# yoseph007/PQA2

Measured on AMD Instinct MI355X. Metric: VMAF frames/sec (vif+adm+motion2 -> SVM), device-resident synthetic YUV pairs, higher is better.
Workload: dtype f32; 1 GPU; 2160p 3840x2160 8-bit, vmaf_4k_v0.6.1, 300 frames/GPU; frames_per_gpu=300, frames_total=300, batch=97, frames_per_launch=75, clips_pipelined=True, parallelism=frame-shard x1, 1-frame motion halo, all-gather of records + of scores

## Files before the change

pqa2_amd/csrc/kernels.h:

```cpp
#pragma once
#include <hip/hip_runtime.h>
#include <stdint.h>

#include <vector>

namespace pqa {

enum Elem : int { ELEM_U8 = 0, ELEM_U16 = 1, ELEM_F32 = 2 };

struct PlaneRun {
  const void* base;
  int64_t row_pitch;
  int64_t frame_pitch;
};

struct MutPlaneRun {
  void* base;
  int64_t row_pitch;
  int64_t frame_pitch;
};

int vif_tile_w(int scale);
constexpr int kVifTileH = 8;
inline int vif_tiles_x(int scale, int w) { return (w + vif_tile_w(scale) - 1) / vif_tile_w(scale); }
inline int vif_tiles_y(int h) { return (h + kVifTileH - 1) / kVifTileH; }

enum : int { VIF_S0_VALU = 0, VIF_S0_AUTO = 1 };
hipError_t launch_vif_stat(hipStream_t stream, int scale, Elem elem, PlaneRun ref, PlaneRun dis, int n_frames,
                           int w, int h, float inv_scale, float gain_limit, int border101, double* partials,
                           MutPlaneRun next_ref, MutPlaneRun next_dis, int s0_mode = VIF_S0_AUTO, int* n_partials = nullptr,
                           int uniform = 1);
hipError_t vif_march_prepare();
int vif_march_partials_max(int w, int h);
int vif_march_table(uint16_t* out, int capacity_halfwords);
void vif_march_shape(int w, int h, int* out6);
bool launch_vif_s0_march(hipStream_t stream, Elem elem, int bits, PlaneRun ref, PlaneRun dis, int n_frames, int w, int h, float gain_limit,
                         int border101, double* partials, MutPlaneRun next_ref, MutPlaneRun next_dis, int* n_partials,
                         hipError_t* err, int uniform = 1);
constexpr int kVifFxPartials = 8;
void vif_fixed_log2_table(uint16_t* out32768);
hipError_t launch_vif_fixed(hipStream_t stream, int scale, int bit_depth, Elem elem, PlaneRun ref, PlaneRun dis,
                            int n_frames, int w, int h, double gain_limit, const uint16_t* log2_lut,
                            long long* partials, MutPlaneRun next_ref, MutPlaneRun next_dis);

constexpr int kAdmTileW = 60, kAdmTileH = 14;
inline int adm_tiles_x(int band_w) { return (band_w + kAdmTileW - 1) / kAdmTileW; }
inline int adm_tiles_y(int band_h) { return (band_h + kAdmTileH - 1) / kAdmTileH; }

enum : int { ADM_TILED = 0, ADM_AUTO = 1, ADM_MARCH = 2 };
hipError_t launch_adm_scale(hipStream_t stream, int scale, Elem elem, PlaneRun ref, PlaneRun dis, int n_frames,
                            int w, int h, float inv_scale, float gain_limit, MutPlaneRun ll_ref,
                            MutPlaneRun ll_dis, double* partials, int mode = ADM_AUTO, int* n_partials = nullptr);
int adm_march_partials(int band_w, int band_h);
bool launch_adm_march(hipStream_t stream, int scale, Elem elem, PlaneRun ref, PlaneRun dis, int n_frames, int w, int h,
                      float inv_scale, float gain_limit, MutPlaneRun ll_ref, MutPlaneRun ll_dis, double* partials,
                      int* n_partials, hipError_t* err);
bool adm_pyramid_takes(Elem elem, int w, int h);
int adm_pyramid_partials(int w, int h);
bool launch_adm_pyramid(hipStream_t stream, Elem elem, PlaneRun ref, PlaneRun dis, int n_frames, int w, int h, float inv_scale,
                        float gain_limit, MutPlaneRun ll_ref, MutPlaneRun ll_dis, double* partials0, double* partials1,
                        int* n_partials, hipError_t* err);
float adm_dwt_quant_step(int lambda, int theta);

constexpr int kAdmFxRows = kAdmTileH + 2;
struct AdmFxScale {
  int scale, band_w, band_h;
  int left, top, right, bottom;
  float rf[3];
  uint32_t i_rf[3];
  int cm_shift_sq[3], cm_shift_sub[3], cm_shift_cub[3], cm_final_q[3];
  int den_shift_sq, den_shift_cub, den_final_q;
  int num_row_shift, den_row_shift;
};
AdmFxScale adm_fixed_scale_params(int scale, int band_w, int band_h);
void adm_fixed_div_table(int32_t* out65537);
void adm_fixed_epilogue(const AdmFxScale& p, const long long acc[6], double* num_out, double* den_out);
hipError_t launch_adm_fixed(hipStream_t stream, int scale, int bit_depth, Elem elem, PlaneRun ref, PlaneRun dis,
                            int n_frames, int w, int h, double gain_limit, const int32_t* div_lut,
                            MutPlaneRun ll_ref, MutPlaneRun ll_dis, long long* partials);

constexpr int kMotionTileW = 252, kMotionTileH = 16;
inline int motion_tiles(int w, int h) {
  return ((w + kMotionTileW - 1) / kMotionTileW) * ((h + kMotionTileH - 1) / kMotionTileH);
}
enum : int { MOTION_TILED = 0, MOTION_AUTO = 1 };
hipError_t launch_motion(hipStream_t stream, Elem elem, PlaneRun ref, const void* prev0, int64_t prev0_row_pitch,
                         int n_frames, int w, int h, float inv_scale, double* partials, int mode = MOTION_AUTO,
                         int* n_partials = nullptr);
int motion_march_partials(int w, int h);
bool launch_motion_march(hipStream_t stream, Elem elem, PlaneRun ref, const void* prev0, int64_t prev0_row_pitch, int n_frames,
                         int w, int h, double* partials, int* n_partials, hipError_t* err);
hipError_t launch_motion_fixed(hipStream_t stream, int bit_depth, Elem elem, PlaneRun ref, const void* prev0,
                               int64_t prev0_row_pitch, int n_frames, int w, int h, unsigned long long* partials);

constexpr int kSseBlocksPerPlane = 256;
hipError_t launch_sse(hipStream_t stream, Elem elem, PlaneRun a, PlaneRun b, int n_frames, int w, int h,
                      unsigned long long* partials);

constexpr int kSsimTileBW = 32, kSsimTileBH = 8;
inline int ssim_tiles(int w, int h) {
  const int ww = (w >> 2) - 1, wh = (h >> 2) - 1;
  if (ww < 1 || wh < 1) return 0;
  return ((ww + kSsimTileBW - 1) / kSsimTileBW) * ((wh + kSsimTileBH - 1) / kSsimTileBH);
}
hipError_t launch_ssim(hipStream_t stream, Elem elem, PlaneRun main, PlaneRun ref, int n_frames, int w, int h,
                       int max_value, double* partials, unsigned long long* sse_partials);

constexpr int kLumaBlocks = 128;
hipError_t launch_luma_stats(hipStream_t stream, Elem elem, PlaneRun luma, int n_frames, int w, int h,
                             unsigned threshold, int gray_bit_depth, unsigned long long* partials,
                             unsigned long long* out);
void luma_gray_map(int bit_depth, float* a, float* b);

struct FinalizeArgs {
// ... 261 lines not shown
```

pqa2_amd/csrc/pqa_api.hip:

```cpp
#include "pqa_ctx.h"

#include <algorithm>
#include <cstdarg>
#include <cstdio>
#include <cstdlib>
#include <mutex>

#include "ingest.h"

using namespace pqa;
using pqa::host::PackPool;
using pqa::host::PackTask;
using pqa::host::run_pack_task;

static thread_local std::string g_create_error;

int pqa::fail(pqa_ctx* c, int code, const char* fmt, ...) {
  char buf[512];
  va_list ap;
  va_start(ap, fmt);
  vsnprintf(buf, sizeof buf, fmt, ap);
  va_end(ap);
  if (c) c->err = buf; else g_create_error = buf;
  return code;
// ... 104 lines not shown
    if (!ref->plane[p] || !dis->plane[p]) return fail(c, PQA_EINVAL, "plane %d pointer is null", p);
  }
  {
    const int rc = check_slots_free(c, first, n);
    if (rc != PQA_OK) return rc;
  }
  c->started = true;
  const PlaneRun rY{ref->plane[0], ref->row_pitch[0] / es, ref->frame_pitch[0] / es};
  const PlaneRun dY{dis->plane[0], dis->row_pitch[0] / es, dis->frame_pitch[0] / es};
  const int w = c->pw[0], h = c->ph[0];
  hipStream_t st = c->stream;
  const bool multi = c->multi_stream && !(c->prof && c->prof_mask == 0xffffffffu);
  hipStream_t st_adm = multi ? c->aux[0] : st, st_misc = multi ? c->aux[1] : st;

  const int k = c->k_sub;
  int e0 = 0, sp_n = n;
  if (k > 1) {
    e0 = (int)((k - first % k) % k);
    sp_n = e0 < n ? (n - e0 + k - 1) / k : 0;
  }
  const bool fork_late = multi && c->multi_stream == 2 && (feat & PQA_FEAT_VIF) && !c->vif_fixed && sp_n > 0;
  if (multi && !fork_late) {
    HIPCHK(c, hipEventRecord(c->fork_ev, st));
    HIPCHK(c, hipStreamWaitEvent(st_adm, c->fork_ev, 0));
    HIPCHK(c, hipStreamWaitEvent(st_misc, c->fork_ev, 0));
  }
  const auto sub = [&](PlaneRun r) {
    return PlaneRun{(const uint8_t*)r.base + (int64_t)e0 * r.frame_pitch * es, r.row_pitch, r.frame_pitch * k};
  };
  const PlaneRun rYs = k > 1 ? sub(rY) : rY, dYs = k > 1 ? sub(dY) : dY;

  const void* p0 = prev;
  int64_t p0_pitch = prev_pitch_bytes;
  if (feat & PQA_FEAT_MOTION) {
    if (!p0 && (c->halo_armed || (c->have_last && c->last_index == first - 1))) {
      p0 = c->last_luma;
      p0_pitch = c->last_luma_pitch;
    }
    if (p0 && p0_pitch % es) return fail(c, PQA_EINVAL, "halo pitch is not a multiple of the sample size");
  }
  int vif_np[4] = {c->vif_tiles[0], c->vif_tiles[1], c->vif_tiles[2], c->vif_tiles[3]};
  int adm_np[4] = {c->adm_tiles[0], c->adm_tiles[1], c->adm_tiles[2], c->adm_tiles[3]};
  int motion_np = c->motion_tiles_n;

  if ((feat & PQA_FEAT_VIF) && sp_n > 0 && c->vif_fixed) {
    PlaneRun cr = rYs, cd = dYs;
    Elem ce = c->elem;
    int cw = w, ch = h;
    for (int s = 0; s < 4; ++s) {
      MutPlaneRun nr{nullptr, 0, 0}, nd{nullptr, 0, 0};
      if (s < 3) {
        Level& L = c->vif_lv[s + 1];
        nr = MutPlaneRun{L.ref, L.pitch, L.frame_pitch};
        nd = MutPlaneRun{L.dis, L.pitch, L.frame_pitch};
      }
      {
        ProfScope ps(c, s, sp_n, st);
        HIPCHK(c, launch_vif_fixed(st, s, (int)c->cfg.bit_depth, ce, cr, cd, sp_n, cw, ch, c->cfg.vif_enhn_gain_limit,
                                   c->vif_lut, c->vif_fx_part[s], nr, nd));
      }
      if (s < 3) {
        Level& L = c->vif_lv[s + 1];
        cr = PlaneRun{L.ref, L.pitch, L.frame_pitch};
        cd = PlaneRun{L.dis, L.pitch, L.frame_pitch};
        ce = ELEM_U16;
        cw = L.w; ch = L.h;
      }
    }
  } else if ((feat & PQA_FEAT_VIF) && sp_n > 0) {
    PlaneRun cr = rYs, cd = dYs;
    Elem ce = c->elem;
    int cw = w, ch = h;
    for (int s = 0; s < 4; ++s) {
      MutPlaneRun nr{nullptr, 0, 0}, nd{nullptr, 0, 0};
      if (s < 3) {
        Level& L = c->vif_lv[s + 1];
        nr = MutPlaneRun{L.ref, L.pitch, L.frame_pitch};
        nd = MutPlaneRun{L.dis, L.pitch, L.frame_pitch};
      }
      {
        ProfScope ps(c, s, sp_n, st);
        HIPCHK(c, launch_vif_stat(st, s, ce, cr, cd, sp_n, cw, ch, c->inv_scale,
                                  (float)c->cfg.vif_enhn_gain_limit, c->cfg.vif_border == PQA_VIF_BORDER_INTEGER,
                                  c->vif_part[s], nr, nd, c->vif_s0_mode, &vif_np[s], c->vif_uniform));
      }
      if (s == 0 && fork_late) {
        HIPCHK(c, hipEventRecord(c->fork_ev, st));
        HIPCHK(c, hipStreamWaitEvent(st_adm, c->fork_ev, 0));
        HIPCHK(c, hipStreamWaitEvent(st_misc, c->fork_ev, 0));
      }
      if (s < 3) {
        Level& L = c->vif_lv[s + 1];
        cr = PlaneRun{L.ref, L.pitch, L.frame_pitch};
        cd = PlaneRun{L.dis, L.pitch, L.frame_pitch};
        ce = ELEM_F32;
        cw = L.w; ch = L.h;
      }
    }
  }
  if ((feat & PQA_FEAT_ADM) && sp_n > 0 && c->adm_fixed) {
    PlaneRun cr = rYs, cd = dYs;
    Elem ce = c->elem;
    int cw = w, ch = h;
    for (int s = 0; s < 4; ++s) {
      MutPlaneRun lr{nullptr, 0, 0}, ld{nullptr, 0, 0};
      if (s < 3) {
        Level& L = c->adm_lv[s + 1];
        lr = MutPlaneRun{L.ref, L.pitch, L.frame_pitch};
        ld = MutPlaneRun{L.dis, L.pitch, L.frame_pitch};
      }
      {
        ProfScope ps(c, 7 + s, sp_n, st_adm);
        HIPCHK(c, launch_adm_fixed(st_adm, s, (int)c->cfg.bit_depth, ce, cr, cd, sp_n, cw, ch,
                                   c->cfg.adm_enhn_gain_limit, c->adm_div_lut, lr, ld, c->adm_fx_part[s]));
      }
      if (s < 3) {
        Level& L = c->adm_lv[s + 1];
        cr = PlaneRun{L.ref, L.pitch, L.frame_pitch};
        cd = PlaneRun{L.dis, L.pitch, L.frame_pitch};
        ce = ELEM_F32;
        cw = L.w; ch = L.h;
      }
    }
  } else if ((feat & PQA_FEAT_ADM) && sp_n > 0) {
    PlaneRun cr = rYs, cd = dYs;
    Elem ce = c->elem;
    int cw = w, ch = h;
    int s = 0;
    if (c->adm_mode == ADM_AUTO) {
      Level& L2 = c->adm_lv[2];
      hipError_t perr = hipSuccess;
      int np = 0;
      ProfScope ps(c, 7, sp_n, st_adm);
      if (launch_adm_pyramid(st_adm, ce, cr, cd, sp_n, cw, ch, c->inv_scale, (float)c->cfg.adm_enhn_gain_limit,
                             MutPlaneRun{L2.ref, L2.pitch, L2.frame_pitch}, MutPlaneRun{L2.dis, L2.pitch, L2.frame_pitch},
                             c->adm_part[0], c->adm_part[1], &np, &perr)) {
        HIPCHK(c, perr);
        adm_np[0] = adm_np[1] = np;
        cr = PlaneRun{L2.ref, L2.pitch, L2.frame_pitch};
        cd = PlaneRun{L2.dis, L2.pitch, L2.frame_pitch};
        ce = ELEM_F32;
        cw = L2.w; ch = L2.h;
        s = 2;
      }
    }
    for (; s < 4; ++s) {
      MutPlaneRun lr{nullptr, 0, 0}, ld{nullptr, 0, 0};
      if (s < 3) {
        Level& L = c->adm_lv[s + 1];
        lr = MutPlaneRun{L.ref, L.pitch, L.frame_pitch};
        ld = MutPlaneRun{L.dis, L.pitch, L.frame_pitch};
      }
      {
        ProfScope ps(c, 7 + s, sp_n, st_adm);
        HIPCHK(c, launch_adm_scale(st_adm, s, ce, cr, cd, sp_n, cw, ch, c->inv_scale,
                                   (float)c->cfg.adm_enhn_gain_limit, lr, ld, c->adm_part[s], c->adm_mode, &adm_np[s]));
      }
      if (s < 3) {
        Level& L = c->adm_lv[s + 1];
        cr = PlaneRun{L.ref, L.pitch, L.frame_pitch};
        cd = PlaneRun{L.dis, L.pitch, L.frame_pitch};
        ce = ELEM_F32;
        cw = L.w; ch = L.h;
      }
    }
  }
  if (feat & PQA_FEAT_MOTION) {
// ... 625 lines not shown
    return fail(nullptr, PQA_EINVAL, "cambi supports bit depth 8 or 10 (got %u)", cfg->bit_depth);
  if ((cfg->features & PQA_FEAT_PSNR_HVS) && cfg->n_planes != 3)
    return fail(nullptr, PQA_EINVAL, "psnr_hvs needs the chroma planes: n_planes must be 3 (got %u)", cfg->n_planes);
  if ((cfg->features & PQA_FEAT_PSNR_HVS) &&
      (((cfg->width + (1u << cfg->chroma_hshift) - 1) >> cfg->chroma_hshift) < 8 ||
       ((cfg->height + (1u << cfg->chroma_vshift) - 1) >> cfg->chroma_vshift) < 8))
    return fail(nullptr, PQA_EINVAL, "psnr_hvs needs every plane >= 8x8 (frame %ux%u, chroma shifts %u, %u)", cfg->width,
                cfg->height, cfg->chroma_hshift, cfg->chroma_vshift);
  if ((cfg->features & PQA_FEAT_XPSNR_HFR) && !(cfg->features & PQA_FEAT_XPSNR))
    return fail(nullptr, PQA_EINVAL, "xpsnr second-order term (PQA_FEAT_XPSNR_HFR) needs PQA_FEAT_XPSNR");
  if (cfg->features & PQA_FEAT_XPSNR) {
    XpsnrGeometry g{};
    xpsnr_geometry((int)cfg->width, (int)cfg->height, (int)((cfg->width + (1u << cfg->chroma_hshift) - 1) >> cfg->chroma_hshift),
                   (int)((cfg->height + (1u << cfg->chroma_vshift) - 1) >> cfg->chroma_vshift), (int)cfg->n_planes,
                   (int)cfg->bit_depth, &g);
    if (g.bv == 2 && ((cfg->width | cfg->height) & 1))
      return fail(nullptr, PQA_EINVAL, "xpsnr needs an even width and height above 2048x1152 (its 2x2 activity; got %ux%u)",
                  cfg->width, cfg->height);
    if (g.nc_blk > g.n_blk || (cfg->n_planes == 3 && g.nc_blk == 0) || g.bsx + 4 > kXpLdsCols)
      return fail(nullptr, PQA_EINVAL, "xpsnr: unsupported block grid for %ux%u (chroma shifts %u, %u)", cfg->width,
                  cfg->height, cfg->chroma_hshift, cfg->chroma_vshift);
  }
  if ((cfg->features & (PQA_FEAT_SITI_REF_FULL | PQA_FEAT_SITI_DIS_FULL)) && !(cfg->features & PQA_FEAT_SITI))
    return fail(nullptr, PQA_EINVAL, "siti range bits (PQA_FEAT_SITI_REF_FULL / _DIS_FULL) need PQA_FEAT_SITI");
  if ((cfg->features & PQA_FEAT_SITI) && cfg->bit_depth != 8 && cfg->bit_depth != 10)
    return fail(nullptr, PQA_EINVAL, "siti supports bit depth 8 or 10 (got %u)", cfg->bit_depth);
  if (cfg->vif_border > PQA_VIF_BORDER_INTEGER || (cfg->fixed_point & ~(uint32_t)PQA_FIXED_ALL))
    return fail(nullptr, PQA_EINVAL, "bad vif_border %u / fixed_point 0x%x", cfg->vif_border, cfg->fixed_point);
  int ndev = 0;
  if (hipGetDeviceCount(&ndev) != hipSuccess || ndev <= 0)
    return fail(nullptr, PQA_EDEVICE, "no HIP device visible (this library has no CPU fallback)");
  if (cfg->device < 0 || cfg->device >= ndev) return fail(nullptr, PQA_EINVAL, "device %d out of range (%d)", cfg->device, ndev);

  pqa_ctx* c = new (std::nothrow) pqa_ctx();
  if (!c) return fail(nullptr, PQA_ENOMEM, "out of host memory");
  c->cfg = *cfg;
  c->device = cfg->device;
  if (cfg->max_batch) {
    c->B = (int)cfg->max_batch;
  } else {
    const int64_t per_frame = 2ll * cfg->width * cfg->height * (cfg->bit_depth > 8 ? 2 : 1);
    c->B = (int)((1536ll << 20) / per_frame);
    if (c->B < 8) c->B = 8;
  }
  if (c->B > 256) c->B = 256;
  c->HB = c->B < 8 ? c->B : 8;
  c->capacity = cfg->result_capacity ? (int)cfg->result_capacity : 16384;
  if (c->capacity < c->B) c->capacity = c->B;
  c->k_sub = cfg->n_subsample > 1 ? (int)cfg->n_subsample : 1;
  if (c->cfg.vif_enhn_gain_limit <= 0) c->cfg.vif_enhn_gain_limit = 100.0;
  if (c->cfg.adm_enhn_gain_limit <= 0) c->cfg.adm_enhn_gain_limit = 100.0;
  c->elem = cfg->bit_depth > 8 ? ELEM_U16 : ELEM_U8;
  c->esize = cfg->bit_depth > 8 ? 2 : 1;
  c->inv_scale = 1.0f / (float)(1 << (cfg->bit_depth - 8));
  c->n_planes = (int)cfg->n_planes;
  c->pw[0] = (int)cfg->width; c->ph[0] = (int)cfg->height;
  for (int p = 1; p < 3; ++p) {
    c->pw[p] = (int)((cfg->width + (1u << cfg->chroma_hshift) - 1) >> cfg->chroma_hshift);
    c->ph[p] = (int)((cfg->height + (1u << cfg->chroma_vshift) - 1) >> cfg->chroma_vshift);
  }

  auto bail = [&](int rc) {
    g_create_error = c->err;
    pqa_destroy(c);
    return rc;
  };
#define CREATE_TRY(expr) do { int rc_ = (expr); if (rc_ != PQA_OK) return bail(rc_); } while (0)
#define CREATE_HIP(expr) do { hipError_t e_ = (expr); if (e_ != hipSuccess) { \
    fail(c, e_ == hipErrorOutOfMemory ? PQA_ENOMEM : PQA_EDEVICE, "%s failed: %s", #expr, hipGetErrorString(e_)); \
    return bail(e_ == hipErrorOutOfMemory ? PQA_ENOMEM : PQA_EDEVICE); } } while (0)

  CREATE_HIP(hipSetDevice(c->device));
  CREATE_HIP(hipStreamCreateWithFlags(&c->own_stream, hipStreamNonBlocking));
  c->stream = c->own_stream;
  {
    const char* e = getenv("PQA_MULTI_STREAM");
    c->multi_stream = (e && e[0] == '1') ? 1 : (e && e[0] == '2') ? 2 : 0;
    const char* t = getenv("PQA_TRACE");
    c->trace = t && t[0] == '1';
    const char* v = getenv("PQA_VIF_MFMA");
    c->vif_s0_mode = (v && v[0] == '0') ? VIF_S0_VALU : VIF_S0_AUTO;
    const char* vu = getenv("PQA_VIF_UNIFORM");
    c->vif_uniform = !(vu && vu[0] == '0');
    const char* am = getenv("PQA_ADM_MARCH");
    const char* ap = getenv("PQA_ADM_PYRAMID");
    c->adm_mode = (am && am[0] == '0') ? ADM_TILED : (ap && ap[0] == '0') ? ADM_MARCH : ADM_AUTO;
    const char* mm = getenv("PQA_MOTION_MARCH");
    c->motion_mode = (mm && mm[0] == '0') ? MOTION_TILED : MOTION_AUTO;
    const char* xm = getenv("PQA_XSSE_MFMA");
    c->xsse_mfma = !(xm && xm[0] == '0');
    const char* tw = getenv("PQA_TEMPORAL_WALK");
    c->temporal_walk = tw && tw[0] == '1';
  }
  for (int i = 0; i < 2; ++i) {
    CREATE_HIP(hipStreamCreateWithFlags(&c->aux[i], hipStreamNonBlocking));
    CREATE_HIP(hipEventCreateWithFlags(&c->join_ev[i], hipEventDisableTiming));
  }
  CREATE_HIP(hipEventCreateWithFlags(&c->fork_ev, hipEventDisableTiming));
  for (int i = 0; i < kBatchEvents; ++i) CREATE_HIP(hipEventCreateWithFlags(&c->batch_ev[i], hipEventDisableTiming));
  try {
    c->ring.init(c->capacity);
  } catch (...) {
    fail(c, PQA_ENOMEM, "out of host memory");
    return bail(PQA_ENOMEM);
  }

  c->vif_fixed = (cfg->features & PQA_FEAT_VIF) && (cfg->fixed_point & PQA_FIXED_VIF);
  c->motion_fixed = (cfg->features & PQA_FEAT_MOTION) && (cfg->fixed_point & PQA_FIXED_MOTION);
  c->adm_fixed = (cfg->features & PQA_FEAT_ADM) && (cfg->fixed_point & PQA_FIXED_ADM);
  if (c->adm_fixed) {
    std::vector<int32_t> lut(65537);
    adm_fixed_div_table(lut.data());
    CREATE_TRY(dev_alloc(c, &c->adm_div_lut, lut.size()));
    CREATE_HIP(hipMemcpy(c->adm_div_lut, lut.data(), lut.size() * sizeof(int32_t), hipMemcpyHostToDevice));
  }
  if ((cfg->features & PQA_FEAT_VIF) && !c->vif_fixed) CREATE_HIP(vif_march_prepare());
  if (c->vif_fixed) {
    std::vector<uint16_t> lut(32768);
    vif_fixed_log2_table(lut.data());
    CREATE_TRY(dev_alloc(c, &c->vif_lut, lut.size()));
    CREATE_HIP(hipMemcpy(c->vif_lut, lut.data(), lut.size() * sizeof(uint16_t), hipMemcpyHostToDevice));
  }
  const int w = c->pw[0], h = c->ph[0], B = c->B;
  int vw = w, vh = h, aw = w, ah = h;
  for (int s = 0; s < 4; ++s) {
    if (s > 0) {
      vw /= 2; vh /= 2;
      aw = (aw + 1) / 2; ah = (ah + 1) / 2;
      Level& V = c->vif_lv[s];
      V.w = vw; V.h = vh; V.pitch = round_up(vw, 16); V.frame_pitch = V.pitch * vh;
      Level& A = c->adm_lv[s];
      A.w = aw; A.h = ah; A.pitch = round_up(aw, 16); A.frame_pitch = A.pitch * ah;
      if (cfg->features & PQA_FEAT_VIF) {
        CREATE_TRY(dev_alloc(c, &V.ref, (size_t)V.frame_pitch * B));
        CREATE_TRY(dev_alloc(c, &V.dis, (size_t)V.frame_pitch * B));
      }
      if (cfg->features & PQA_FEAT_ADM) {
        CREATE_TRY(dev_alloc(c, &A.ref, (size_t)A.frame_pitch * B));
        CREATE_TRY(dev_alloc(c, &A.dis, (size_t)A.frame_pitch * B));
      }
    }
    if (vw < 2 || vh < 2) { fail(c, PQA_EINVAL, "frame too small for 4 VIF scales"); return bail(PQA_EINVAL); }
    c->vif_tiles[s] = vif_tiles_x(s, vw) * vif_tiles_y(vh);
    if (s == 0) {
      const int mp = vif_march_partials_max(vw, vh);
      c->vif_part_cap0 = c->vif_tiles[0] > mp ? c->vif_tiles[0] : mp;
    }
    const int bw = (aw + 1) / 2, bh = (ah + 1) / 2;
    c->adm_tiles[s] = adm_tiles_x(bw) * adm_tiles_y(bh);
    const int left = (int)(bw * 0.1 - 0.5), top = (int)(bh * 0.1 - 0.5);
    c->adm_area[s] = (float)((bh - 2 * top) * (bw - 2 * left));
    if ((cfg->features & PQA_FEAT_VIF) && !c->vif_fixed)
      CREATE_TRY(dev_alloc(c, &c->vif_part[s], (size_t)(s == 0 ? c->vif_part_cap0 : c->vif_tiles[s]) * 2 * B));
    if ((cfg->features & PQA_FEAT_VIF) && c->vif_fixed)
      CREATE_TRY(dev_alloc(c, &c->vif_fx_part[s], (size_t)c->vif_tiles[s] * kVifFxPartials * B));
    c->adm_fx[s] = adm_fixed_scale_params(s, bw, bh);
    if ((cfg->features & PQA_FEAT_ADM) && !c->adm_fixed) {
      int mp = adm_march_partials(bw, bh);
      if (s < 2 && adm_pyramid_takes(c->elem, w, h)) { const int pp = adm_pyramid_partials(w, h); mp = pp > mp ? pp : mp; }
      CREATE_TRY(dev_alloc(c, &c->adm_part[s], (size_t)(c->adm_tiles[s] > mp ? c->adm_tiles[s] : mp) * 6 * B));
    }
    if ((cfg->features & PQA_FEAT_ADM) && c->adm_fixed)
      CREATE_TRY(dev_alloc(c, &c->adm_fx_part[s], (size_t)c->adm_tiles[s] * kAdmFxRows * 6 * B));
  }
  c->motion_tiles_n = motion_tiles(w, h);
  if (cfg->features & PQA_FEAT_MOTION) {
// ... 662 lines not shown
```

pqa2_amd/csrc/pqa_ctx.h:

```cpp
#pragma once
#include "../../include/pqa_vmaf.h"

#include <atomic>
#include <cstring>
#include <memory>
#include <string>
#include <thread>
#include <vector>

#include "host_pack.h"
#include "host_ring.h"
#include "host_stage.h"
#include "kernels.h"

namespace pqa {

struct Level {
  int w = 0, h = 0;
  int64_t pitch = 0, frame_pitch = 0;
  float* ref = nullptr;
  float* dis = nullptr;
};

struct Half {
// ... 80 lines not shown
  int ms_tiles[pqa::kMsScales] = {};
  double* fs_part = nullptr;
  int fs_tiles = 0, fs_box = 1;
  int ssf_sb = 0;
  double* ciede_part = nullptr;
  int ciede_tiles_n = 0;
  pqa::CambiParams cambi_prm{};
  pqa::CambiWork cambi_wk{};
  int cambi_sb = 0;
  double* ext2 = nullptr;
  pqa::PsnrHvsGeometry phv_geo{};
  double* phv_part = nullptr;
  double* ext3 = nullptr;
  pqa::XpsnrGeometry xp_geo{};
  unsigned long long* xp_blk = nullptr;
  double* xp_w = nullptr;
  uint8_t* xp_hist[2] = {nullptr, nullptr};
  int64_t xp_hist_idx[2] = {-1, -1};
  int64_t xp_hist_pitch = 0;
  uint8_t* xp_prev = nullptr;
  int64_t xp_last = -1;
  int xp_armed = -1;
  double* ext4 = nullptr;
  double* st_part = nullptr;
  uint8_t* st_hist[2] = {nullptr, nullptr};
  int64_t st_hist_idx[2] = {-1, -1};
  int64_t st_hist_pitch = 0;
  bool st_armed[2] = {false, false};
  double* ext5 = nullptr;
  unsigned long long* ig_part = nullptr;
  uint8_t* ig_hist[3] = {nullptr, nullptr, nullptr};
  int64_t ig_hist_pitch[3] = {0, 0, 0};
  int64_t ig_hist_idx = -1;
  bool ig_armed = false;
  uint32_t black_thr = 0;
  bool started = false;
  uint8_t* ig_anchor[3] = {nullptr, nullptr, nullptr};
  uint8_t* ig_stage = nullptr;
  size_t ig_stage_off[3] = {0, 0, 0}, ig_stage_bytes = 0;
  unsigned long long* ig_out = nullptr;
  unsigned long long* luma_part = nullptr;
  unsigned long long* luma_out = nullptr;
  pqa::Half luma_half[2];
  int64_t luma_pitch = 0;
  int LB = 0;
  bool luma_ready = false;
  uint32_t luma_gray = PQA_GRAY_LUMA;
  bool xsse_mfma = true;
  bool temporal_walk = false;
  pqa::RsCached rs_cache[pqa::kRsCached];
  int rs_next = 0;
  uint8_t* side_pin[2] = {nullptr, nullptr};
  size_t side_pin_cap[2] = {0, 0};
  void* side_buf[pqa::kSideBufs] = {};
  size_t side_cap[pqa::kSideBufs] = {};
  uint8_t* last_luma = nullptr;
  int64_t last_luma_pitch = 0;
  int64_t last_index = -1;
  bool have_last = false, halo_armed = false;
  pqa::Half half[2];
  int cur_half = 0, pending = 0;
  int64_t pending_first = 0;
  size_t slot_bytes = 0;
  size_t plane_off[2][3] = {};
  int64_t slot_row_pitch[3] = {};
  bool staging_ready = false;
  std::thread pin_thread;
  hipError_t pin_err = hipSuccess;
  uint8_t* surf_dev = nullptr;
  std::unique_ptr<pqa::host::PackPool> pack_pool;
  bool pack_pool_tried = false;
  std::vector<pqa::host::PackTask> pack_tasks;
  pqa::host::RecordRing ring;
  hipEvent_t batch_ev[pqa::kBatchEvents] = {};
  uint64_t batch_ev_seq[pqa::kBatchEvents] = {};
  uint64_t batch_seq = 0;
  uint64_t done_seq = 0;
  std::atomic<int> cancelled{0};
  std::string err;
  std::vector<void*> allocs;
  int multi_stream = 0;
  int vif_s0_mode = pqa::VIF_S0_AUTO;
  int vif_uniform = 1;
  int adm_mode = pqa::ADM_AUTO;
  int motion_mode = pqa::MOTION_AUTO;
  bool trace = false;
  bool prof = false;
  uint32_t prof_mask = 0xffffffffu;
  std::vector<pqa::ProfEv> evs;
  double prof_ms[PQA_PROF_KERNELS] = {};
  uint64_t prof_n[PQA_PROF_KERNELS] = {}, prof_frames[PQA_PROF_KERNELS] = {};
};

namespace pqa {

int fail(pqa_ctx* c, int code, const char* fmt, ...);

#define HIPCHK(c, expr)                                                                          \
  do {                                                                                           \
    hipError_t e_ = (expr);                                                                      \
    if (e_ != hipSuccess)                                                                        \
      return pqa::fail((c), e_ == hipErrorOutOfMemory ? PQA_ENOMEM : PQA_EDEVICE, "%s failed: %s", #expr, \
                  hipGetErrorString(e_));                                                        \
  } while (0)

template <typename T>
int dev_alloc(pqa_ctx* c, T** out, size_t count) {
  void* p = nullptr;
  if (count == 0) count = 1;
  HIPCHK(c, hipMalloc(&p, count * sizeof(T)));
  c->allocs.push_back(p);
  *out = (T*)p;
  return PQA_OK;
}

}
```

pqa2_amd/csrc/vif.hip:

```cpp
#include <cstring>
#include <mutex>
#include <vector>

#include <cstdio>
#include "kernels.h"
#include "pqa_device.h"

namespace pqa {

namespace {

struct Taps {
  float f[17];
};

static Taps gaussian_taps(int n) {
  Taps t{};
  double v[17], sum = 0.0;
  const double sigma = n / 5.0;
  for (int k = 0; k < n; ++k) {
    const double d = k - n / 2;
    v[k] = exp(-0.5 * d * d / (sigma * sigma));
    sum += v[k];
  }
  for (int k = 0; k < n; ++k) t.f[k] = (float)(v[k] / sum);
  return t;
}

struct TapPairs {
  f2 vt[18];
  f2 ht[17];
  f2 dt[9];
};

static TapPairs tap_pairs(const Taps& t, int n, const Taps* next, int n_next) {
  TapPairs p{};
  if (next)
    for (int k = 0; k < n_next; ++k) p.dt[k] = f2{next->f[k], next->f[k]};
  for (int k = 0; k <= n; ++k) {
    p.vt[k].x = k < n ? t.f[k] : 0.0f;
    p.vt[k].y = k > 0 ? t.f[k - 1] : 0.0f;
  }
  for (int k = 0; k < n; ++k) p.ht[k] = f2{t.f[k], t.f[k]};
  return p;
}

struct VifStatArgs {
  const void* ref;
  const void* dis;
  int64_t row_pitch_r, frame_pitch_r, row_pitch_d, frame_pitch_d;
  int w, h, tiles_x, n_tiles;
  int fold_w, fold_h;
  float inv_scale, gain_limit;
  double* partials;
  float* dst_ref;
  float* dst_dis;
  int64_t dst_row_pitch_r, dst_frame_pitch_r, dst_row_pitch_d, dst_frame_pitch_d;
  TapPairs taps;
  int uniform;
};

constexpr int kP2 = 258;


template <int N, int TW, int ND>
__device__ __forceinline__ void vif_hstat(const VifStatArgs& a, const f2* sv ,
                                          const f2* sd , double* red, int fr, int tile, int x0, int y0) {
  constexpr int R = N / 2, TH = kVifTileH, NSEG = TW / 4, NRP = TH / 2;
  constexpr int RD = ND / 2;
  const int tid = threadIdx.x;
  fr = __builtin_amdgcn_readfirstlane(fr); tile = __builtin_amdgcn_readfirstlane(tile);
  x0 = __builtin_amdgcn_readfirstlane(x0); y0 = __builtin_amdgcn_readfirstlane(y0);
  if (ND) {
    const int ox0 = x0 >> 1, oy0 = y0 >> 1, ow = a.w >> 1, oh = a.h >> 1;
    float* __restrict__ tr = a.dst_ref + ((int64_t)fr * a.dst_frame_pitch_r + (int64_t)oy0 * a.dst_row_pitch_r + ox0);
    float* __restrict__ td = a.dst_dis + ((int64_t)fr * a.dst_frame_pitch_d + (int64_t)oy0 * a.dst_row_pitch_d + ox0);
    const unsigned rp_r = (unsigned)a.dst_row_pitch_r, rp_d = (unsigned)a.dst_row_pitch_d;
#pragma unroll
    for (int round = 0; round < 2; ++round) {
      const int item = tid + round * kBlock;
      const int oc = item & 127, orow = item >> 7;
      if (oc < TW / 2 && (ox0 + oc < ow && oy0 + orow < oh)) {
        f2 acc = f2{0.0f, 0.0f};
#pragma unroll
        for (int k = 0; k < ND; ++k) acc = __builtin_elementwise_fma(a.taps.dt[k], sd[orow * kP2 + 2 * oc + (R - RD) + k], acc);
        *reinterpret_cast<float*>(reinterpret_cast<char*>(tr) + ((unsigned)orow * rp_r + (unsigned)oc) * 4u) = acc.x;
        *reinterpret_cast<float*>(reinterpret_cast<char*>(td) + ((unsigned)orow * rp_d + (unsigned)oc) * 4u) = acc.y;
      }
    }
  }

  const int wave = tid >> 6, lane = tid & 63;
  const int rp = lane & 3, sl = lane >> 2;
  const int seg = 2 * (sl & 3) + (wave & 1) + 8 * (sl >> 2) + 32 * (wave >> 1);
  float num = 0.0f, den = 0.0f;
  if (seg < NSEG) {
    constexpr int NCOL = 4 + N - 1, NREAD = (NCOL + 1) / 2;
    f2 out[5][4];
#pragma unroll
    for (int s = 0; s < 5; ++s) {
      f2 in[2 * NREAD];
      const f4* p = reinterpret_cast<const f4*>(&sv[(s * NRP + rp) * kP2 + seg * 4]);
#pragma unroll
      for (int q = 0; q < NREAD; ++q) {
        const f4 v = p[q];
        in[2 * q] = f2{v.x, v.y};
        in[2 * q + 1] = f2{v.z, v.w};
      }
#pragma unroll
      for (int o = 0; o < 4; ++o) out[s][o] = f2{0.0f, 0.0f};
#pragma unroll
      for (int k = 0; k < N; ++k)
#pragma unroll
        for (int o = 0; o < 4; ++o) out[s][o] = __builtin_elementwise_fma(a.taps.ht[k], in[o + k], out[s][o]);
      __builtin_amdgcn_sched_barrier(0);
    }
    const float sigma_nsq = 2.0f, eps = 1.0e-10f, sigma_max_inv = 4.0f / (255.0f * 255.0f);
    const int gyA = y0 + 2 * rp;
    const bool vrow[2] = {gyA < a.h, gyA + 1 < a.h};
    f2 num2 = f2{0.0f, 0.0f}, den2 = f2{0.0f, 0.0f};
    f2 pn = f2{1.0f, 1.0f}, qn = f2{1.0f, 1.0f}, pd = f2{1.0f, 1.0f};
    f2 s1v[4];
    bool any_low = false;
#pragma unroll
    for (int o = 0; o < 4; ++o) {
      const f2 mu1 = out[0][o];
      s1v[o] = out[2][o] - mu1 * mu1;
      const bool lx = s1v[o].x < sigma_nsq, ly = s1v[o].y < sigma_nsq;
      any_low = any_low || lx || ly;
    }
    const bool cols_in = x0 + seg * 4 + 4 <= a.w;
    const bool rows_in = a.uniform && y0 + TH <= a.h;
    const bool none_low = __builtin_amdgcn_ballot_w64(!cols_in || any_low) == 0ull;
    if (rows_in && none_low) {
#pragma unroll
      for (int o = 0; o < 4; ++o) {
        const f2 mu1 = out[0][o], mu2 = out[1][o];
        const f2 s1 = s1v[o];
        f2 s2 = out[3][o] - mu2 * mu2;
        const f2 s12 = out[4][o] - mu1 * mu2;
        s2 = f2{fmaxf(s2.x, 0.0f), fmaxf(s2.y, 0.0f)};
        const f2 grcp = f2{fast_rcp(s1.x), fast_rcp(s1.y)};
        f2 g = s12 * grcp;
        g = __builtin_elementwise_fma(__builtin_elementwise_fma(-g, s1, s12), grcp, g);
        f2 sv = s2 - g * s12;
        sv = f2{fmaxf(sv.x, eps), fmaxf(sv.y, eps)};
        g = f2{__builtin_amdgcn_fmed3f(g.x, 0.0f, a.gain_limit), __builtin_amdgcn_fmed3f(g.y, 0.0f, a.gain_limit)};
        const f2 svn = sv + f2{sigma_nsq, sigma_nsq};
        const f2 narg = __builtin_elementwise_fma(g * g, s1, svn);
        const f2 darg = __builtin_elementwise_fma(s1, f2{1.0f / sigma_nsq, 1.0f / sigma_nsq}, f2{1.0f, 1.0f});
        pn *= narg;
        qn *= svn;
        pd *= darg;
        __builtin_amdgcn_sched_barrier(0);
      }
      num = (fast_log2(pn.x) - fast_log2(qn.x)) + (fast_log2(pn.y) - fast_log2(qn.y));
      den = fast_log2(pd.x) + fast_log2(pd.y);
    } else {
#pragma unroll
      for (int o = 0; o < 4; ++o) {
        const bool vcol = (x0 + seg * 4 + o) < a.w;
        const f2 mu1 = out[0][o], mu2 = out[1][o];
        const f2 s1 = s1v[o];
        f2 s2 = out[3][o] - mu2 * mu2;
        const f2 s12 = out[4][o] - mu1 * mu2;
        s2 = f2{fmaxf(s2.x, 0.0f), fmaxf(s2.y, 0.0f)};
        const bool vx = vcol && vrow[0], vy = vcol && vrow[1];
        const bool hx = vx && !(s1.x < sigma_nsq), hy = vy && !(s1.y < sigma_nsq);
        const bool lx = vx && (s1.x < sigma_nsq), ly = vy && (s1.y < sigma_nsq);
        const f2 s1h = f2{hx ? s1.x : 0.0f, hy ? s1.y : 0.0f};
        const f2 gden = s1h + f2{eps, eps};
        const f2 grcp = f2{fast_rcp(gden.x), fast_rcp(gden.y)};
        f2 g = s12 * grcp;
        g = __builtin_elementwise_fma(__builtin_elementwise_fma(-g, gden, s12), grcp, g);
        f2 sv = s2 - g * s12;
        sv = f2{fmaxf(sv.x, eps), fmaxf(sv.y, eps)};
        g = f2{__builtin_amdgcn_fmed3f(g.x, 0.0f, a.gain_limit), __builtin_amdgcn_fmed3f(g.y, 0.0f, a.gain_limit)};
        const f2 svn = sv + f2{sigma_nsq, sigma_nsq};
        const f2 narg = __builtin_elementwise_fma(g * g, s1h, svn);
        const f2 darg = __builtin_elementwise_fma(s1h, f2{1.0f / sigma_nsq, 1.0f / sigma_nsq}, f2{1.0f, 1.0f});
        const f2 low = __builtin_elementwise_fma(s2, f2{-sigma_max_inv, -sigma_max_inv}, f2{1.0f, 1.0f});
        pn *= narg;
        qn *= svn;
        pd *= darg;
        const f2 wl = f2{lx ? 1.0f : 0.0f, ly ? 1.0f : 0.0f};
        num2 = __builtin_elementwise_fma(wl, low, num2);
        den2 += wl;
        __builtin_amdgcn_sched_barrier(0);
      }
      num = (num2.x + num2.y) + ((fast_log2(pn.x) - fast_log2(qn.x)) + (fast_log2(pn.y) - fast_log2(qn.y)));
      den = (den2.x + den2.y) + (fast_log2(pd.x) + fast_log2(pd.y));
    }
  }
  {
    const float part[2] = {num, den};
    double v[2];
    block_sum_f32<2>(part, v, red);
    if (tid == 0) {
      double* out = a.partials + ((int64_t)fr * a.n_tiles + tile) * 2;
      out[0] = v[0];
      out[1] = v[1];
    }
  }
}

template <typename T, int N, int TW, int ND>
__global__ __launch_bounds__(kBlock, 3) void vif_stat_kernel(const VifStatArgs a) {
  constexpr int R = N / 2, TH = kVifTileH, COLS = TW + N - 1, NSEG = TW / 4, S = 8, NIN = S + N - 1;
  constexpr int RD = ND / 2;
  static_assert(ND == 0 || RD <= R, "decimation window must sit inside the statistic window");
  static_assert(COLS <= 256 && COLS <= kP2, "one column per thread");
  static_assert(TW % 4 == 0 && NSEG <= 64 && TH == S, "segment map");
  __shared__ f2 sv[5][TH / 2][kP2];
  __shared__ f2 sd[ND ? TH / 2 : 1][ND ? kP2 : 1];
  __shared__ double red[12];

  const int tile = xcd_remap(blockIdx.x, a.n_tiles);
  const int tx = tile % a.tiles_x, ty = tile / a.tiles_x;
  const int fr = blockIdx.y;
  const T* __restrict__ ref = (const T*)a.ref + (int64_t)fr * a.frame_pitch_r;
  const T* __restrict__ dis = (const T*)a.dis + (int64_t)fr * a.frame_pitch_d;
  const int x0 = tx * TW, y0 = ty * TH;
  const int tid = threadIdx.x;

  {
    const int col = tid;
    constexpr int seg = 0;
    if (col < COLS) {
      const unsigned gx = (unsigned)mirror_fold(x0 - R + col, a.w, a.fold_w);
      const unsigned pitch_r = (unsigned)a.row_pitch_r, pitch_d = (unsigned)a.row_pitch_d;
      const auto rsrc_r = make_rsrc(ref, (unsigned)a.h * pitch_r * (unsigned)sizeof(T));
      const auto rsrc_d = make_rsrc(dis, (unsigned)a.h * pitch_d * (unsigned)sizeof(T));
      f2 acc[S / 2][5];
#pragma unroll
      for (int p = 0; p < S / 2; ++p)
#pragma unroll
        for (int s = 0; s < 5; ++s) acc[p][s] = f2{0.0f, 0.0f};
      f2 dacc[S / 2];
#pragma unroll
      for (int q = 0; q < S / 2; ++q) dacc[q] = f2{0.0f, 0.0f};
#ifndef PQA_VIF_G
#define PQA_VIF_G 12
#endif
      constexpr int G = PQA_VIF_G, NG = (NIN + G - 1) / G;
      T rn[G], dn[G];
      auto issue = [&](int g) {
#pragma unroll
        for (int i = 0; i < G; ++i) {
          const int j = g * G + i;
          if (j < NIN) {
            const unsigned gy = (unsigned)mirror_fold(y0 + seg * S - R + j, a.h, a.fold_h);
            rn[i] = buf_load<T>(rsrc_r, gx, gy * pitch_r);
            dn[i] = buf_load<T>(rsrc_d, gx, gy * pitch_d);
          }
        }
      };
      issue(0);
#pragma unroll
      for (int g = 0; g < NG; ++g) {
        T rc[G], dc[G];
#pragma unroll
        for (int i = 0; i < G; ++i) { rc[i] = rn[i]; dc[i] = dn[i]; }
        if (g + 1 < NG) issue(g + 1);
#pragma unroll
        for (int i = 0; i < G; ++i) {
          const int j = g * G + i;
          if (j < NIN) {
            const f2 x = PixIO<T>::pair(rc[i], dc[i], a.inv_scale);
            const f2 xx = x * x;
            const float r = x.x, d = x.y, rr = xx.x, dd = xx.y, rd = x.x * x.y;
            if (ND) {
#pragma unroll
              for (int q = 0; q < S / 2; ++q) {
                const int kd = j - (2 * q + R - RD);
                if (kd >= 0 && kd < ND) dacc[q] = __builtin_elementwise_fma(a.taps.dt[kd], x, dacc[q]);
              }
            }
#pragma unroll
            for (int p = 0; p < S / 2; ++p) {
              const int k = j - 2 * p;
              if (k >= 0 && k <= N) {
                const f2 c = a.taps.vt[k];
                acc[p][0] = __builtin_elementwise_fma(c, f2{r, r}, acc[p][0]);
                acc[p][1] = __builtin_elementwise_fma(c, f2{d, d}, acc[p][1]);
                acc[p][2] = __builtin_elementwise_fma(c, f2{rr, rr}, acc[p][2]);
                acc[p][3] = __builtin_elementwise_fma(c, f2{dd, dd}, acc[p][3]);
                acc[p][4] = __builtin_elementwise_fma(c, f2{rd, rd}, acc[p][4]);
              }
            }
          }
        }
        __builtin_amdgcn_sched_barrier(0);
      }
#pragma unroll
      for (int p = 0; p < S / 2; ++p)
#pragma unroll
        for (int s = 0; s < 5; ++s) sv[s][seg * (S / 2) + p][col] = acc[p][s];
      if (ND) {
#pragma unroll
        for (int q = 0; q < S / 2; ++q) sd[seg * (S / 2) + q][col] = dacc[q];
      }
    }
  }
  __syncthreads();

  vif_hstat<N, TW, ND>(a, &sv[0][0][0], &sd[0][0], red, fr, tile, x0, y0);
}


template <int N, int TW, int ND>
hipError_t launch_stat_n(hipStream_t stream, Elem elem, const VifStatArgs& a, int n_frames) {
  const dim3 grid(a.n_tiles, n_frames), block(kBlock);
  switch (elem) {
    case ELEM_U8: hipLaunchKernelGGL((vif_stat_kernel<uint8_t, N, TW, ND>), grid, block, 0, stream, a); break;
    case ELEM_U16: hipLaunchKernelGGL((vif_stat_kernel<uint16_t, N, TW, ND>), grid, block, 0, stream, a); break;
    case ELEM_F32: hipLaunchKernelGGL((vif_stat_kernel<float, N, TW, ND>), grid, block, 0, stream, a); break;
  }
  return hipGetLastError();
}

constexpr int kVifN[4] = {17, 9, 5, 3};
constexpr int kVifTW[4] = {240, 248, 252, 252};

}

int vif_tile_w(int scale) { return kVifTW[scale]; }

hipError_t launch_vif_stat(hipStream_t stream, int scale, Elem elem, PlaneRun ref, PlaneRun dis, int n_frames,
                           int w, int h, float inv_scale, float gain_limit, int border101, double* partials,
                           MutPlaneRun next_ref, MutPlaneRun next_dis, int s0_mode, int* n_partials, int uniform) {
  if (n_partials) *n_partials = vif_tiles_x(scale, w) * vif_tiles_y(h);
  if (n_frames <= 0) return hipSuccess;
  const int bits = elem == ELEM_U8 ? 8 : (elem == ELEM_U16 && inv_scale == 0.25f) ? 10 : (elem == ELEM_U16 && inv_scale == 0.0625f) ? 12 : 0;
  if (scale == 0 && bits && s0_mode == VIF_S0_AUTO && next_ref.base && next_dis.base) {
    hipError_t err = hipSuccess;
    if (launch_vif_s0_march(stream, elem, bits, ref, dis, n_frames, w, h, gain_limit, border101, partials, next_ref, next_dis, n_partials, &err, uniform))
      return err;
    if (n_partials) *n_partials = vif_tiles_x(scale, w) * vif_tiles_y(h);
  }
  VifStatArgs a{};
  a.ref = ref.base; a.dis = dis.base;
  a.row_pitch_r = ref.row_pitch; a.frame_pitch_r = ref.frame_pitch;
  a.row_pitch_d = dis.row_pitch; a.frame_pitch_d = dis.frame_pitch;
  a.w = w; a.h = h;
  a.fold_w = 2 * w - (border101 ? 2 : 1); a.fold_h = 2 * h - (border101 ? 2 : 1);
  a.tiles_x = vif_tiles_x(scale, w);
  a.n_tiles = a.tiles_x * vif_tiles_y(h);
  a.inv_scale = inv_scale; a.gain_limit = gain_limit;
  a.uniform = uniform;
  a.partials = partials;
  a.dst_ref = (float*)next_ref.base; a.dst_dis = (float*)next_dis.base;
  a.dst_row_pitch_r = next_ref.row_pitch; a.dst_frame_pitch_r = next_ref.frame_pitch;
  a.dst_row_pitch_d = next_dis.row_pitch; a.dst_frame_pitch_d = next_dis.frame_pitch;
  const Taps cur = gaussian_taps(kVifN[scale]);
  const Taps nxt = scale < 3 ? gaussian_taps(kVifN[scale + 1]) : Taps{};
  a.taps = tap_pairs(cur, kVifN[scale], scale < 3 ? &nxt : nullptr, scale < 3 ? kVifN[scale + 1] : 0);
  if (scale < 3 && (!a.dst_ref || !a.dst_dis)) return hipErrorInvalidValue;
  switch (scale) {
    case 0: return launch_stat_n<17, 240, 9>(stream, elem, a, n_frames);
    case 1: return launch_stat_n<9, 248, 5>(stream, elem, a, n_frames);
    case 2: return launch_stat_n<5, 252, 3>(stream, elem, a, n_frames);
    case 3: return launch_stat_n<3, 252, 0>(stream, elem, a, n_frames);
  }
  return hipErrorInvalidValue;
}

}
```

Measured before the change: 22880 frames/s.

## Stage VIF statistic planes through LDS in two phases to raise occupancy

The VIF stat kernel now writes only two of the five vertical-filtered planes to shared memory, runs the horizontal pass on them, then reuses the same buffers for the remaining three planes after a barrier. This shrinks the per-block LDS footprint from 5 (or 6) plane buffers to 3, and the launch bounds now ask for 4 or 5 blocks per CU instead of 3. The cost is an extra barrier and keeping the vertical accumulators live in registers across the first horizontal pass. The old single-phase path stays selectable through an environment variable.

```diff
diff --git a/pqa2_amd/csrc/kernels.h b/pqa2_amd/csrc/kernels.h
--- a/pqa2_amd/csrc/kernels.h
+++ b/pqa2_amd/csrc/kernels.h
@@ -29,7 +29,7 @@
 hipError_t launch_vif_stat(hipStream_t stream, int scale, Elem elem, PlaneRun ref, PlaneRun dis, int n_frames,
                            int w, int h, float inv_scale, float gain_limit, int border101, double* partials,
                            MutPlaneRun next_ref, MutPlaneRun next_dis, int s0_mode = VIF_S0_AUTO, int* n_partials = nullptr,
-                           int uniform = 1);
+                           int uniform = 1, int phases = 1);
 hipError_t vif_march_prepare();
 int vif_march_partials_max(int w, int h);
 int vif_march_table(uint16_t* out, int capacity_halfwords);
diff --git a/pqa2_amd/csrc/pqa_api.hip b/pqa2_amd/csrc/pqa_api.hip
--- a/pqa2_amd/csrc/pqa_api.hip
+++ b/pqa2_amd/csrc/pqa_api.hip
@@ -210,7 +210,7 @@
         ProfScope ps(c, s, sp_n, st);
         HIPCHK(c, launch_vif_stat(st, s, ce, cr, cd, sp_n, cw, ch, c->inv_scale,
                                   (float)c->cfg.vif_enhn_gain_limit, c->cfg.vif_border == PQA_VIF_BORDER_INTEGER,
-                                  c->vif_part[s], nr, nd, c->vif_s0_mode, &vif_np[s], c->vif_uniform));
+                                  c->vif_part[s], nr, nd, c->vif_s0_mode, &vif_np[s], c->vif_uniform, c->vif_phases));
       }
       if (s == 0 && fork_late) {
         HIPCHK(c, hipEventRecord(c->fork_ev, st));
@@ -1002,6 +1002,8 @@
     c->vif_s0_mode = (v && v[0] == '0') ? VIF_S0_VALU : VIF_S0_AUTO;
     const char* vu = getenv("PQA_VIF_UNIFORM");
     c->vif_uniform = !(vu && vu[0] == '0');
+    const char* vp = getenv("PQA_VIF_PHASES");
+    c->vif_phases = !(vp && vp[0] == '0');
     const char* am = getenv("PQA_ADM_MARCH");
     const char* ap = getenv("PQA_ADM_PYRAMID");
     c->adm_mode = (am && am[0] == '0') ? ADM_TILED : (ap && ap[0] == '0') ? ADM_MARCH : ADM_AUTO;
diff --git a/pqa2_amd/csrc/pqa_ctx.h b/pqa2_amd/csrc/pqa_ctx.h
--- a/pqa2_amd/csrc/pqa_ctx.h
+++ b/pqa2_amd/csrc/pqa_ctx.h
@@ -186,6 +186,7 @@
   int multi_stream = 0;
   int vif_s0_mode = pqa::VIF_S0_AUTO;
   int vif_uniform = 1;
+  int vif_phases = 1;
   int adm_mode = pqa::ADM_AUTO;
   int motion_mode = pqa::MOTION_AUTO;
   bool trace = false;
diff --git a/pqa2_amd/csrc/vif.hip b/pqa2_amd/csrc/vif.hip
--- a/pqa2_amd/csrc/vif.hip
+++ b/pqa2_amd/csrc/vif.hip
@@ -64,13 +64,9 @@
 
 
 template <int N, int TW, int ND>
-__device__ __forceinline__ void vif_hstat(const VifStatArgs& a, const f2* sv ,
-                                          const f2* sd , double* red, int fr, int tile, int x0, int y0) {
-  constexpr int R = N / 2, TH = kVifTileH, NSEG = TW / 4, NRP = TH / 2;
-  constexpr int RD = ND / 2;
+__device__ __forceinline__ void vif_decimate(const VifStatArgs& a, const f2* sd , int fr, int x0, int y0) {
+  constexpr int R = N / 2, RD = ND / 2;
   const int tid = threadIdx.x;
-  fr = __builtin_amdgcn_readfirstlane(fr); tile = __builtin_amdgcn_readfirstlane(tile);
-  x0 = __builtin_amdgcn_readfirstlane(x0); y0 = __builtin_amdgcn_readfirstlane(y0);
   if (ND) {
     const int ox0 = x0 >> 1, oy0 = y0 >> 1, ow = a.w >> 1, oh = a.h >> 1;
     float* __restrict__ tr = a.dst_ref + ((int64_t)fr * a.dst_frame_pitch_r + (int64_t)oy0 * a.dst_row_pitch_r + ox0);
@@ -89,32 +85,48 @@
       }
     }
   }
-
+}
+
+__device__ __forceinline__ void vif_lane_map(int& rp, int& seg) {
+  const int tid = threadIdx.x;
   const int wave = tid >> 6, lane = tid & 63;
-  const int rp = lane & 3, sl = lane >> 2;
-  const int seg = 2 * (sl & 3) + (wave & 1) + 8 * (sl >> 2) + 32 * (wave >> 1);
+  const int sl = lane >> 2;
+  rp = lane & 3;
+  seg = 2 * (sl & 3) + (wave & 1) + 8 * (sl >> 2) + 32 * (wave >> 1);
+}
+
+template <int N, int S0, int S1>
+__device__ __forceinline__ void vif_hpass(const VifStatArgs& a, const f2* pl , int rp, int seg,
+                                          f2 (&out)[5][4]) {
+  constexpr int NRP = kVifTileH / 2;
+  constexpr int NCOL = 4 + N - 1, NREAD = (NCOL + 1) / 2;
+#pragma unroll
+  for (int s = S0; s < S1; ++s) {
+    f2 in[2 * NREAD];
+    const f4* p = reinterpret_cast<const f4*>(&pl[((s - S0) * NRP + rp) * kP2 + seg * 4]);
+#pragma unroll
+    for (int q = 0; q < NREAD; ++q) {
+      const f4 v = p[q];
+      in[2 * q] = f2{v.x, v.y};
+      in[2 * q + 1] = f2{v.z, v.w};
+    }
+#pragma unroll
+    for (int o = 0; o < 4; ++o) out[s][o] = f2{0.0f, 0.0f};
+#pragma unroll
+    for (int k = 0; k < N; ++k)
+#pragma unroll
+      for (int o = 0; o < 4; ++o) out[s][o] = __builtin_elementwise_fma(a.taps.ht[k], in[o + k], out[s][o]);
+    __builtin_amdgcn_sched_barrier(0);
+  }
+}
+
+template <int N, int TW>
+__device__ __forceinline__ void vif_statistic(const VifStatArgs& a, const f2 (&out)[5][4], double* red, int fr, int tile,
+                                              int x0, int y0, int rp, int seg) {
+  constexpr int TH = kVifTileH, NSEG = TW / 4;
+  const int tid = threadIdx.x;
   float num = 0.0f, den = 0.0f;
   if (seg < NSEG) {
-    constexpr int NCOL = 4 + N - 1, NREAD = (NCOL + 1) / 2;
-    f2 out[5][4];
-#pragma unroll
-    for (int s = 0; s < 5; ++s) {
-      f2 in[2 * NREAD];
-      const f4* p = reinterpret_cast<const f4*>(&sv[(s * NRP + rp) * kP2 + seg * 4]);
-#pragma unroll
-      for (int q = 0; q < NREAD; ++q) {
-        const f4 v = p[q];
-        in[2 * q] = f2{v.x, v.y};
-        in[2 * q + 1] = f2{v.z, v.w};
-      }
-#pragma unroll
-      for (int o = 0; o < 4; ++o) out[s][o] = f2{0.0f, 0.0f};
-#pragma unroll
-      for (int k = 0; k < N; ++k)
-#pragma unroll
-        for (int o = 0; o < 4; ++o) out[s][o] = __builtin_elementwise_fma(a.taps.ht[k], in[o + k], out[s][o]);
-      __builtin_amdgcn_sched_barrier(0);
-    }
     const float sigma_nsq = 2.0f, eps = 1.0e-10f, sigma_max_inv = 4.0f / (255.0f * 255.0f);
     const int gyA = y0 + 2 * rp;
     const bool vrow[2] = {gyA < a.h, gyA + 1 < a.h};
@@ -204,15 +216,20 @@
   }
 }
 
-template <typename T, int N, int TW, int ND>
-__global__ __launch_bounds__(kBlock, 3) void vif_stat_kernel(const VifStatArgs a) {
+constexpr int vif_waves(int n, int ph) { return !ph ? 3 : n > 9 ? 4 : 5; }
+#ifndef PQA_VIF_LDS_EXTRA
+#define PQA_VIF_LDS_EXTRA 0
+#endif
+
+template <typename T, int N, int TW, int ND, int PH>
+__global__ __launch_bounds__(kBlock, vif_waves(N, PH)) void vif_stat_kernel(const VifStatArgs a) {
   constexpr int R = N / 2, TH = kVifTileH, COLS = TW + N - 1, NSEG = TW / 4, S = 8, NIN = S + N - 1;
   constexpr int RD = ND / 2;
   static_assert(ND == 0 || RD <= R, "decimation window must sit inside the statistic window");
   static_assert(COLS <= 256 && COLS <= kP2, "one column per thread");
   static_assert(TW % 4 == 0 && NSEG <= 64 && TH == S, "segment map");
-  __shared__ f2 sv[5][TH / 2][kP2];
-  __shared__ f2 sd[ND ? TH / 2 : 1][ND ? kP2 : 1];
+  constexpr int NPL = PH ? 3 : (ND ? 6 : 5), SD = !ND ? 0 : PH ? 2 : 5;
+  __shared__ f2 pl[NPL][TH / 2][kP2];
   __shared__ double red[12];
 
   const int tile = xcd_remap(blockIdx.x, a.n_tiles);
@@ -223,19 +240,19 @@
   const int x0 = tx * TW, y0 = ty * TH;
   const int tid = threadIdx.x;
 
+  const int col = tid;
+  f2 acc[S / 2][5];
+#pragma unroll
+  for (int p = 0; p < S / 2; ++p)
+#pragma unroll
+    for (int s = 0; s < 5; ++s) acc[p][s] = f2{0.0f, 0.0f};
   {
-    const int col = tid;
     constexpr int seg = 0;
     if (col < COLS) {
       const unsigned gx = (unsigned)mirror_fold(x0 - R + col, a.w, a.fold_w);
       const unsigned pitch_r = (unsigned)a.row_pitch_r, pitch_d = (unsigned)a.row_pitch_d;
       const auto rsrc_r = make_rsrc(ref, (unsigned)a.h * pitch_r * (unsigned)sizeof(T));
       const auto rsrc_d = make_rsrc(dis, (unsigned)a.h * pitch_d * (unsigned)sizeof(T));
-      f2 acc[S / 2][5];
-#pragma unroll
-      for (int p = 0; p < S / 2; ++p)
-#pragma unroll
-        for (int s = 0; s < 5; ++s) acc[p][s] = f2{0.0f, 0.0f};
       f2 dacc[S / 2];
 #pragma unroll
       for (int q = 0; q < S / 2; ++q) dacc[q] = f2{0.0f, 0.0f};
@@ -295,28 +312,51 @@
 #pragma unroll
       for (int p = 0; p < S / 2; ++p)
 #pragma unroll
-        for (int s = 0; s < 5; ++s) sv[s][seg * (S / 2) + p][col] = acc[p][s];
+        for (int s = 0; s < (PH ? 2 : 5); ++s) pl[s][p][col] = acc[p][s];
       if (ND) {
 #pragma unroll
-        for (int q = 0; q < S / 2; ++q) sd[seg * (S / 2) + q][col] = dacc[q];
+        for (int q = 0; q < S / 2; ++q) pl[SD][q][col] = dacc[q];
       }
     }
   }
   __syncthreads();
 
-  vif_hstat<N, TW, ND>(a, &sv[0][0][0], &sd[0][0], red, fr, tile, x0, y0);
-}
-
+  const int sfr = __builtin_amdgcn_readfirstlane(fr), stile = __builtin_amdgcn_readfirstlane(tile);
+  const int sx0 = __builtin_amdgcn_readfirstlane(x0), sy0 = __builtin_amdgcn_readfirstlane(y0);
+  vif_decimate<N, TW, ND>(a, &pl[SD][0][0], sfr, sx0, sy0);
+  int rp, hseg;
+  vif_lane_map(rp, hseg);
+  f2 out[5][4];
+  if (hseg < NSEG) vif_hpass<N, 0, (PH ? 2 : 5)>(a, &pl[0][0][0], rp, hseg, out);
+  if (PH) {
+    __syncthreads();
+    if (col < COLS) {
+#pragma unroll
+      for (int p = 0; p < S / 2; ++p)
+#pragma unroll
+        for (int s = 2; s < 5; ++s) pl[s - 2][p][col] = acc[p][s];
+    }
+    __syncthreads();
+    if (hseg < NSEG) vif_hpass<N, 2, 5>(a, &pl[0][0][0], rp, hseg, out);
+  }
+  vif_statistic<N, TW>(a, out, red, sfr, stile, sx0, sy0, rp, hseg);
+}
+
+template <int N, int TW, int ND, int PH>
+hipError_t launch_stat_ph(hipStream_t stream, Elem elem, const VifStatArgs& a, int n_frames) {
+  const dim3 grid(a.n_tiles, n_frames), block(kBlock);
+  constexpr unsigned extra = PH ? PQA_VIF_LDS_EXTRA : 0;
+  switch (elem) {
+    case ELEM_U8: hipLaunchKernelGGL((vif_stat_kernel<uint8_t, N, TW, ND, PH>), grid, block, extra, stream, a); break;
+    case ELEM_U16: hipLaunchKernelGGL((vif_stat_kernel<uint16_t, N, TW, ND, PH>), grid, block, extra, stream, a); break;
+    case ELEM_F32: hipLaunchKernelGGL((vif_stat_kernel<float, N, TW, ND, PH>), grid, block, extra, stream, a); break;
+  }
+  return hipGetLastError();
+}
 
 template <int N, int TW, int ND>
-hipError_t launch_stat_n(hipStream_t stream, Elem elem, const VifStatArgs& a, int n_frames) {
-  const dim3 grid(a.n_tiles, n_frames), block(kBlock);
-  switch (elem) {
-    case ELEM_U8: hipLaunchKernelGGL((vif_stat_kernel<uint8_t, N, TW, ND>), grid, block, 0, stream, a); break;
-    case ELEM_U16: hipLaunchKernelGGL((vif_stat_kernel<uint16_t, N, TW, ND>), grid, block, 0, stream, a); break;
-    case ELEM_F32: hipLaunchKernelGGL((vif_stat_kernel<float, N, TW, ND>), grid, block, 0, stream, a); break;
-  }
-  return hipGetLastError();
+hipError_t launch_stat_n(hipStream_t stream, Elem elem, const VifStatArgs& a, int n_frames, int phases) {
+  return phases ? launch_stat_ph<N, TW, ND, 1>(stream, elem, a, n_frames) : launch_stat_ph<N, TW, ND, 0>(stream, elem, a, n_frames);
 }
 
 constexpr int kVifN[4] = {17, 9, 5, 3};
@@ -328,7 +368,7 @@
 
 hipError_t launch_vif_stat(hipStream_t stream, int scale, Elem elem, PlaneRun ref, PlaneRun dis, int n_frames,
                            int w, int h, float inv_scale, float gain_limit, int border101, double* partials,
-                           MutPlaneRun next_ref, MutPlaneRun next_dis, int s0_mode, int* n_partials, int uniform) {
+                           MutPlaneRun next_ref, MutPlaneRun next_dis, int s0_mode, int* n_partials, int uniform, int phases) {
   if (n_partials) *n_partials = vif_tiles_x(scale, w) * vif_tiles_y(h);
   if (n_frames <= 0) return hipSuccess;
   const int bits = elem == ELEM_U8 ? 8 : (elem == ELEM_U16 && inv_scale == 0.25f) ? 10 : (elem == ELEM_U16 && inv_scale == 0.0625f) ? 12 : 0;
@@ -357,10 +397,10 @@
   a.taps = tap_pairs(cur, kVifN[scale], scale < 3 ? &nxt : nullptr, scale < 3 ? kVifN[scale + 1] : 0);
   if (scale < 3 && (!a.dst_ref || !a.dst_dis)) return hipErrorInvalidValue;
   switch (scale) {
-    case 0: return launch_stat_n<17, 240, 9>(stream, elem, a, n_frames);
-    case 1: return launch_stat_n<9, 248, 5>(stream, elem, a, n_frames);
-    case 2: return launch_stat_n<5, 252, 3>(stream, elem, a, n_frames);
-    case 3: return launch_stat_n<3, 252, 0>(stream, elem, a, n_frames);
+    case 0: return launch_stat_n<17, 240, 9>(stream, elem, a, n_frames, phases);
+    case 1: return launch_stat_n<9, 248, 5>(stream, elem, a, n_frames, phases);
+    case 2: return launch_stat_n<5, 252, 3>(stream, elem, a, n_frames, phases);
+    case 3: return launch_stat_n<3, 252, 0>(stream, elem, a, n_frames, phases);
   }
   return hipErrorInvalidValue;
 }
```

Result: slower. 22590 frames/s (-1.3%).
